# microsoft/AI2BMD

Hardware: NVIDIA H100
Metric: MD steps/sec (higher is better)
Workload: dtype f32

## Files before the change

### ai2bmd_b200/csrc/k_edge_tc.cuh

```cuda
#pragma once
#include "k_edge.cuh"
#include "tc_common.cuh"

namespace vb {

constexpr int TC_TE = 128;
constexpr int TC_STAGES = 2;
constexpr int TC_MAX_STAGES = 3;
constexpr int TC_SLABS = D / tc::SLAB_K;
static_assert((TC_SLABS & (TC_SLABS - 1)) == 0, "tc_slab rotates the slab order with a mask: TC_SLABS must be a power of two");
constexpr int TC_MAXJOBS = 12;
constexpr int TC_LT = D + LDS_PAD;
typedef float TcRow[TC_LT];

struct TcJob {
    const float* img;
    int accumulate;
};

struct TcShared {
    alignas(1024) uint8_t ring[TC_STAGES][tc::STAGE_BYTES];
    alignas(16) float tile[TC_TE][TC_LT];
    alignas(16) float abuf[TC_TE][TC_LT];
    EdgeMeta<TC_TE> meta;
// ... 29 lines not shown
    const int stage = k % NS, job = (k / TC_SLABS) % sh.njobs, s = tc_slab(k % TC_SLABS);
    const char* src = reinterpret_cast<const char*>(sh.jobs[job].img) + (size_t)s * tc::STAGE_BYTES;
    tc::mbar_arrive_expect_tx(&sh.b_full[stage], tc::STAGE_BYTES);
    tc::tma_load_1d(tc_stage_ptr(sh, stage), src, tc::STAGE_BYTES, &sh.b_full[stage]);
}

}


namespace vb {

constexpr int TC2_CWARPS = 16;
constexpr int TC2_CTHREADS = TC2_CWARPS * 32;
constexpr int TC2_THREADS = TC2_CTHREADS;
constexpr int TC2_NGRP = TC2_CTHREADS / D;

struct EdgeTcArgs {
    int layer;
    ModelW mw;
    Workspace ws;
    TcJob jobs[TC_MAXJOBS];
    int njobs;
    int tile_rows;
    unsigned long long* tl;
};
constexpr int TC_TL_SLOTS = 64;
#define TC_TL(k) do { if (a.tl != nullptr && blockIdx.x == 0 && it == 0 && threadIdx.x == 0) a.tl[k] = (unsigned long long)clock64(); } while (0)

__device__ __forceinline__ void csync() { asm volatile("bar.sync 1, %0;" ::"n"(TC2_CTHREADS) : "memory"); }

constexpr int TC2_WS_THREADS = TC2_CTHREADS / 2;
__device__ __forceinline__ bool tc2_is_mma_warp(int warp) { return ((warp >> 2) & 1) == 0; }
__device__ __forceinline__ void gather_sync() { asm volatile("bar.sync 2, %0;" ::"n"(TC2_WS_THREADS) : "memory"); }
__device__ __forceinline__ void handoff_arrive(int id) { asm volatile("bar.arrive %0, %1;" ::"r"(id), "n"(TC2_CTHREADS) : "memory"); }
__device__ __forceinline__ void handoff_wait(int id) { asm volatile("bar.sync %0, %1;" ::"r"(id), "n"(TC2_CTHREADS) : "memory"); }

template <int ROWS>
struct TcRing {
    static constexpr int NS = tc_nstages(ROWS);
    int next = 0;
};

template <int ROWS>
__device__ __forceinline__ void tc2_setup(TcShared& sh, const TcRing<ROWS>&, const TcJob* jobs, int njobs, int ntiles) {
    constexpr int NS = TcRing<ROWS>::NS;
    if (threadIdx.x == 0) {
        for (int s = 0; s < NS; s++) { tc::mbar_init(&sh.b_full[s], 1); sh.released[s] = 0; }
        tc::mbar_init(&sh.b_tile, TC2_CWARPS);
        sh.jobs = jobs; sh.njobs = njobs; sh.nslabs = ntiles * njobs * TC_SLABS;
        tc::fence_barrier_init();
    }
    __syncthreads();
    if (threadIdx.x == 0)
        for (int k = 0; k < NS; k++) tc_issue<NS>(sh, k);
}

template <int NS, int NW>
__device__ __forceinline__ void tc2_release(TcShared& sh, int k, int lane) {
    __syncwarp();
    if (lane == 0) {
        const uint32_t before = tc::atom_add_acq_rel(&sh.released[k % NS], 1u);
        if (before % NW == NW - 1) tc_issue<NS>(sh, k + NS);
    }
}

__device__ __forceinline__ void tc2_tile_to_a(TcShared& sh, int rows) {
// ... 201 lines not shown
    const int trows = min(ROWS, max(16, a.tile_rows));
    const int ntiles_total = (E + trows - 1) / trows;
    const int my_tiles = ((int)blockIdx.x < ntiles_total) ? (ntiles_total - (int)blockIdx.x + (int)gridDim.x - 1) / (int)gridDim.x : 0;
    if (a.tl != nullptr && blockIdx.x == 0 && threadIdx.x == 0) a.tl[0] = (unsigned long long)clock64();
    TcRing<ROWS> ring;
    tc2_setup(sh, ring, a.jobs, a.njobs, my_tiles);
    if (a.tl != nullptr && blockIdx.x == 0 && threadIdx.x == 0) a.tl[1] = (unsigned long long)clock64();

    float acc[32];
    const float* __restrict__ Fin = ws.F[l];
    float* __restrict__ Fout = upd ? ws.F[l + 1] : nullptr;
    const float* __restrict__ QKV = ws.QKV[l];
    const float* __restrict__ VN = ws.VN[l];
    const float* __restrict__ TU = ws.TU[l];
    float* __restrict__ P1 = ws.P1[l];
    float* __restrict__ SP = ws.SP[l];
    float* __restrict__ ATT = ws.ATT[l];
    for (int it = 0; it < my_tiles; it++) {
        const uint32_t tpar = (uint32_t)(it & 1);
        const int e0 = ((int)blockIdx.x + it * (int)gridDim.x) * trows;
        const int nvalid = min(trows, E - e0);
        {
            constexpr int RW = ROWS / TC2_CWARPS;
            const int w0 = warp * RW, wn = max(0, min(RW, nvalid - w0));
            if (lane == 0) {
                if (wn > 0) tc::mbar_arrive_expect_tx(&sh.b_tile, (uint32_t)wn * D * 4);
                else tc::mbar_arrive(&sh.b_tile);
            }
            __syncwarp();
            if (lane < wn) tc::tma_load_1d(&sh.abuf[w0 + lane][0], Fin + (size_t)(e0 + w0 + lane) * D, D * 4, &sh.b_tile);
        }
        load_edge_meta<TC_TE, TC2_CTHREADS>(sh.meta, ws, e0, nvalid);
        if constexpr (SMALL) {
            enum : int { H_DK = 3, H_ATT, H_DV, H_F, H_M, H_EU };
            TcRow* const xb = tc_aux(sh);
            csync();
            if (tc2_is_mma_warp(warp)) {
                tc::mbar_wait(&sh.b_tile, tpar);
                TC_TL(2);
                tc2_mma<ROWS, true>(sh, ring, sh.abuf, acc, a.jobs[J_DK].accumulate, warp, lane, nvalid);
                tc2_acc_to(sh.tile, acc, warp, lane, nvalid);
                handoff_arrive(H_DK);
                TC_TL(4);
                tc2_mma<ROWS, true>(sh, ring, sh.abuf, acc, a.jobs[J_DV].accumulate, warp, lane, nvalid);
                TC_TL(7);
                handoff_wait(H_ATT);
                tc2_acc_to(xb, acc, warp, lane, nvalid);
                handoff_arrive(H_DV);
                TC_TL(8);
                if (upd) {
                    tc2_mma<ROWS, true>(sh, ring, sh.abuf, acc, a.jobs[J_F].accumulate, warp, lane, nvalid);
                    tc2_acc_to(sh.tile, acc, warp, lane, nvalid);
                    handoff_arrive(H_F);
                    TC_TL(11);
                }
                handoff_wait(H_M);
                TC_TL(3);
                tc2_mma<ROWS, true>(sh, ring, xb, acc, a.jobs[J_S1].accumulate, warp, lane, nvalid);
                tc2_acc_to(sh.abuf, acc, warp, lane, nvalid);
                TC_TL(13);
                if (threadIdx.x == 0 && it + 1 < my_tiles) {
                    const int en = ((int)blockIdx.x + (it + 1) * (int)gridDim.x) * trows;
                    tc::tma_prefetch_l2(Fin + (size_t)en * D, (uint32_t)min(trows, E - en) * D * 4);
                }
                tc2_mma<ROWS, true>(sh, ring, xb, acc, a.jobs[J_S2].accumulate, warp, lane, nvalid);
                TC_TL(16);
                if (upd) handoff_wait(H_EU);
// ... 197 lines not shown
            }
            TC_TL(12);
            float bnd[2][3] = {{0.f, 0.f, 0.f}, {0.f, 0.f, 0.f}};
            tc2_mma(sh, ring, sh.abuf, acc, a.jobs[J_S1].accumulate, warp, lane, nvalid);
            TC_TL(13);
            csync();
            tc2_acc_to(sh.tile, acc, warp, lane, nvalid);
            csync();
            TC_TL(14);
            tc_fwd_s1(sh, ws, lw, VN, SP, sh.tile, e0, nvalid, cch, grp, TC2_NGRP, bnd);
            TC_TL(15);
            if (threadIdx.x == 0 && it + 1 < my_tiles) {
                const int en = ((int)blockIdx.x + (it + 1) * (int)gridDim.x) * trows;
                tc::tma_prefetch_l2(Fin + (size_t)en * D, (uint32_t)min(trows, E - en) * D * 4);
            }
            tc2_mma(sh, ring, sh.abuf, acc, a.jobs[J_S2].accumulate, warp, lane, nvalid);
            TC_TL(16);
            csync();
            tc2_acc_to(sh.tile, acc, warp, lane, nvalid);
            csync();
            TC_TL(17);
            tc_fwd_s2(sh, ws, lw, SP, sh.tile, e0, nvalid, cch, grp, TC2_NGRP, bnd);
            TC_TL(18);
        }
        csync();
    }
    if (a.tl != nullptr && blockIdx.x == 0 && threadIdx.x == 0) a.tl[31] = (unsigned long long)clock64();
}

}

namespace vb {

template <int ROWS>
__global__ void __launch_bounds__(TC2_THREADS, 1) edge_bwd_tc_kernel(const __grid_constant__ EdgeTcArgs a) {
    pdl_entry();
    extern __shared__ __align__(1024) uint8_t dyn_raw[];
    TcShared& sh = *tc_shared_base(dyn_raw);
    const Workspace& ws = a.ws;
    const int l = a.layer;
    const bool upd = (l < L - 1);
    const int J_G3A = 0, J_G3B = 1, J_G4DV = 2, J_G4DK = 3, J_G4F = 4;
    const int J_LAST = upd ? J_G4F : J_G4DK;
    constexpr int RPW = ROWS / TC2_CWARPS;
    constexpr int RB4 = (RPW % 4 == 0) ? 4 : 2;
    constexpr bool SMALL = ROWS <= 64;
    constexpr int RBM = SMALL ? 2 : RB4;
    const int warp = threadIdx.x >> 5, lane = threadIdx.x & 31, col = lane * 4, hd = lane >> 2;
    const int E = ws.rowptr[ws.N];
    const int trows = min(ROWS, max(16, a.tile_rows));
    const int ntiles_total = (E + trows - 1) / trows;
    const int my_tiles = ((int)blockIdx.x < ntiles_total) ? (ntiles_total - (int)blockIdx.x + (int)gridDim.x - 1) / (int)gridDim.x : 0;
    if (a.tl != nullptr && blockIdx.x == 0 && threadIdx.x == 0) a.tl[0] = (unsigned long long)clock64();
    TcRing<ROWS> ring;
    tc2_setup(sh, ring, a.jobs, a.njobs, my_tiles);
    if (a.tl != nullptr && blockIdx.x == 0 && threadIdx.x == 0) a.tl[1] = (unsigned long long)clock64();

    float acc[32];
    const float* __restrict__ QKV = ws.QKV[l];
    const float* __restrict__ VN = ws.VN[l];
    const float* __restrict__ TU = ws.TU[l];
    const float* __restrict__ P1 = ws.P1[l];
    const float* __restrict__ SP = ws.SP[l];
    const float* __restrict__ ATT = ws.ATT[l];
    const int cch = threadIdx.x & (D - 1), grp = threadIdx.x >> 7;
    for (int it = 0; it < my_tiles; it++) {
        const int e0 = ((int)blockIdx.x + it * (int)gridDim.x) * trows;
        const int nvalid = min(trows, E - e0);
        const int rpw = (nvalid + TC2_CWARPS - 1) / TC2_CWARPS, r0 = warp * rpw;
        load_edge_meta<TC_TE, TC2_CTHREADS>(sh.meta, ws, e0, nvalid);
        csync();
        TC_TL(2);
        if constexpr (SMALL) {
#pragma unroll 1
            for (int rb = 0; rb < RPW; rb += RB4) {
                if (rb >= rpw) break;
                float4 sp[RB4][2], gM[RB4][3], vn[RB4][3];
#pragma unroll
                for (int u = 0; u < RB4; u++) {
                    const int row = r0 + rb + u;
                    const size_t e = (size_t)(e0 + ((rb + u < rpw && row < nvalid) ? row : 0));
                    const size_t i3 = (size_t)sh.meta.dst[row] * 3, j3 = (size_t)sh.meta.src[row] * 3;
                    sp[u][0] = ldg4(SP + e * 2 * D + col);
                    sp[u][1] = ldg4(SP + e * 2 * D + D + col);
#pragma unroll
                    for (int s = 0; s < 3; s++) { gM[u][s] = ldg4(ws.GVEC + (i3 + s) * D + col); vn[u][s] = ldg4(VN + (j3 + s) * D + col); }
                }
#pragma unroll
                for (int u = 0; u < RB4; u++) {
                    const int row = r0 + rb + u;
                    const bool mine = rb + u < rpw, ok = (mine && row < nvalid);
                    const size_t j3 = (size_t)sh.meta.src[row] * 3;
                    const float4 dd = sh.meta.d[row];
                    const float4 s1 = silu4(sp[u][0]), s2 = silu4(sp[u][1]);
                    const float4 gs1 = gM[u][0] * vn[u][0] + gM[u][1] * vn[u][1] + gM[u][2] * vn[u][2];
                    const float gx_ = warp_sum(hsum4(gM[u][0] * s2)), gy_ = warp_sum(hsum4(gM[u][1] * s2)), gz_ = warp_sum(hsum4(gM[u][2] * s2));
                    if (mine) {
                        st4(&sh.abuf[row][col], ok ? gs1 * dsilu4(sp[u][0]) : f4s(0.f));
                        st4(&sh.tile[row][col], ok ? (gM[u][0] * dd.x + gM[u][1] * dd.y + gM[u][2] * dd.z) * dsilu4(sp[u][1]) : f4s(0.f));
                        if (lane == 0) { sh.eacc[row][1] = gx_; sh.eacc[row][2] = gy_; sh.eacc[row][3] = gz_; }
                    }
                    if (ok) {
                        red4(ws.GVNMSG + (j3 + 0) * D + col, gM[u][0] * s1);
                        red4(ws.GVNMSG + (j3 + 1) * D + col, gM[u][1] * s1);
                        red4(ws.GVNMSG + (j3 + 2) * D + col, gM[u][2] * s1);
                    }
                }
            }
            TC_TL(3);
        } else {
#pragma unroll 1
            for (int rb = 0; rb < RPW; rb += RB4) {
                if (rb >= rpw) break;
                float4 sp[RB4], gM[RB4][3], vn[RB4][3];
#pragma unroll
                for (int u = 0; u < RB4; u++) {
                    const int row = r0 + rb + u;
                    const size_t e = (size_t)(e0 + ((rb + u < rpw && row < nvalid) ? row : 0));
                    const size_t i3 = (size_t)sh.meta.dst[row] * 3, j3 = (size_t)sh.meta.src[row] * 3;
                    sp[u] = ldg4(SP + e * 2 * D + col);
#pragma unroll
                    for (int s = 0; s < 3; s++) { gM[u][s] = ldg4(ws.GVEC + (i3 + s) * D + col); vn[u][s] = ldg4(VN + (j3 + s) * D + col); }
                }
#pragma unroll
                for (int u = 0; u < RB4; u++) {
                    const int row = r0 + rb + u;
                    const bool ok = (rb + u < rpw && row < nvalid);
                    const size_t j3 = (size_t)sh.meta.src[row] * 3;
                    const float4 s1 = silu4(sp[u]);
                    const float4 gs1 = gM[u][0] * vn[u][0] + gM[u][1] * vn[u][1] + gM[u][2] * vn[u][2];
                    if (rb + u < rpw) st4(&sh.abuf[row][col], ok ? gs1 * dsilu4(sp[u]) : f4s(0.f));
                    if (ok) {
                        red4(ws.GVNMSG + (j3 + 0) * D + col, gM[u][0] * s1);
                        red4(ws.GVNMSG + (j3 + 1) * D + col, gM[u][1] * s1);
                        red4(ws.GVNMSG + (j3 + 2) * D + col, gM[u][2] * s1);
                    }
                }
            }
            TC_TL(3);
#pragma unroll 4
            for (int r = 0; r < RPW; r++) {
                if (r >= rpw) break;
                const int row = r0 + r;
                const bool ok = (r < rpw && row < nvalid);
                const size_t e = (size_t)(e0 + (ok ? row : 0));
                const size_t i3 = (size_t)sh.meta.dst[row] * 3;
                const float4 dd = sh.meta.d[row];
                const float4 sp = ldg4(SP + e * 2 * D + D + col);
                const float4 s2 = silu4(sp);
                const float4 gM0 = ldg4(ws.GVEC + (i3 + 0) * D + col), gM1 = ldg4(ws.GVEC + (i3 + 1) * D + col),
                             gM2 = ldg4(ws.GVEC + (i3 + 2) * D + col);
                const float gx_ = warp_sum(hsum4(gM0 * s2)), gy_ = warp_sum(hsum4(gM1 * s2)), gz_ = warp_sum(hsum4(gM2 * s2));
                if (lane == 0) { sh.eacc[row][1] = gx_; sh.eacc[row][2] = gy_; sh.eacc[row][3] = gz_; }
                st4(&sh.tile[row][col], ok ? (gM0 * dd.x + gM1 * dd.y + gM2 * dd.z) * dsilu4(sp) : f4s(0.f));
            }
            TC_TL(5);
        }
        csync();
        tc2_mma(sh, ring, sh.abuf, acc, a.jobs[J_G3A].accumulate, warp, lane, nvalid);
        TC_TL(6);
        if constexpr (!SMALL) {
            tc2_tile_to_a(sh, nvalid);
            TC_TL(7);
        }
        tc2_mma(sh, ring, SMALL ? sh.tile : sh.abuf, acc, a.jobs[J_G3B].accumulate, warp, lane, nvalid);
        TC_TL(8);
        csync();
        tc2_acc_to(sh.tile, acc, warp, lane, nvalid);
        csync();
        TC_TL(9);
#pragma unroll 1
        for (int rb = 0; rb < RPW; rb += RBM) {
            if (rb >= rpw) break;
            float4 gxa[RBM], vjr[RBM], pdvr[RBM];
            float avr[RBM];
#pragma unroll
            for (int u = 0; u < RBM; u++) {
                const int row = r0 + rb + u;
                const size_t e = (size_t)(e0 + ((rb + u < rpw && row < nvalid) ? row : 0));
                gxa[u] = load_gxa(ws, (size_t)sh.meta.dst[row], col);
                vjr[u] = ldg4(QKV + (size_t)sh.meta.src[row] * 3 * D + 2 * D + col);
                pdvr[u] = ldg4(P1 + e * 3 * D + D + col);
                avr[u] = (rb + u < rpw && row < nvalid) ? __ldg(ATT + e * H + hd) : 0.f;
            }
#pragma unroll
            for (int u = 0; u < RBM; u++) {
                const int row = r0 + rb + u;
                const bool ok = (rb + u < rpw && row < nvalid);
                const size_t j = sh.meta.src[row];
                const float Ce = sh.meta.C[row];
                const float av = avr[u], sa = silu_(av), A = sa * Ce;
                const bool mine = rb + u < rpw;
                const float4 gm = mine ? ld4(&sh.tile[row][col]) + gxa[u] : f4s(0.f);
                const float4 dv = silu4(pdvr[u]);
                if (mine) st4(&sh.abuf[row][col], ok ? gm * vjr[u] * A * dsilu4(pdvr[u]) : f4s(0.f));
                const float gA = quad_sum(hsum4(gm * vjr[u] * dv));
                if (mine && (lane & 3) == 0) sh.gattn[row][hd] = gA * Ce * dsilu_(av);
                const float gc = warp_sum((lane & 3) == 0 ? gA * sa : 0.f);
                if (mine && lane == 0) sh.eacc[row][0] = gc;
                if (ok) red4(ws.GQKV + j * 3 * D + 2 * D + col, gm * dv * A);
            }
        }
        TC_TL(10);
        csync();
#pragma unroll 1
        for (int rb = 0; rb < RPW; rb += RB4) {
            if (rb >= rpw) break;
            float4 pdkr[RB4], qir[RB4], kjr[RB4];
#pragma unroll
            for (int u = 0; u < RB4; u++) {
                const int row = r0 + rb + u;
                const size_t e = (size_t)(e0 + ((rb + u < rpw && row < nvalid) ? row : 0));
                pdkr[u] = ldg4(P1 + e * 3 * D + col);
                qir[u] = ldg4(QKV + (size_t)sh.meta.dst[row] * 3 * D + col);
                kjr[u] = ldg4(QKV + (size_t)sh.meta.src[row] * 3 * D + D + col);
            }
#pragma unroll
            for (int u = 0; u < RB4; u++) {
                const int row = r0 + rb + u;
                const bool ok = (rb + u < rpw && row < nvalid);
                const size_t j = sh.meta.src[row];
                const float4 dk = silu4(pdkr[u]);
                const float gav = sh.gattn[row][hd];
                if (rb + u < rpw) st4(&sh.tile[row][col], ok ? qir[u] * kjr[u] * gav * dsilu4(pdkr[u]) : f4s(0.f));
                if (SMALL && rb + u < rpw) st4(&tc_aux(sh)[row][col], kjr[u] * dk * gav);
                if (ok) red4(ws.GQKV + j * 3 * D + D + col, qir[u] * dk * gav);
            }
        }
        TC_TL(12);
        csync();
        tc2_mma(sh, ring, sh.abuf, acc, a.jobs[J_G4DV].accumulate, warp, lane, nvalid);
        TC_TL(13);
        if constexpr (!SMALL) {
            tc2_tile_to_a(sh, nvalid);
            TC_TL(14);
            csync();
#pragma unroll 4
            for (int r = 0; r < RPW; r++) {
                if (r >= rpw) break;
                const int row = r0 + r;
                const size_t e = (size_t)(e0 + ((r < rpw && row < nvalid) ? row : 0));
                const float4 dk = silu4(ldg4(P1 + e * 3 * D + col));
                const float4 kj = ldg4(QKV + (size_t)sh.meta.src[row] * 3 * D + D + col);
                st4(&sh.tile[row][col], kj * dk * sh.gattn[row][hd]);
            }
            csync();
        }
        {
            const TcRow* const gqb = SMALL ? tc_aux(sh) : sh.tile;
            const int i_first = sh.meta.dst[0], i_last = sh.meta.dst[nvalid - 1];
            for (int i = i_first + grp; i <= i_last; i += TC2_NGRP) {
                const int q0 = ws.rowptr[i], q1 = ws.rowptr[i + 1];
                const int lo = max(q0, e0) - e0, hi = min(q1, e0 + nvalid) - e0;
                float gq = 0.f;
                for (int r = lo; r < hi; r++) gq += gqb[r][cch];
                if (q0 >= e0 && q1 <= e0 + nvalid) ws.GQKV[(size_t)i * 3 * D + cch] = gq;
                else atomicAdd(ws.GQKV + (size_t)i * 3 * D + cch, gq);
            }
        }
        TC_TL(15);
        if (upd) {
            TcRow* const gpfb = SMALL ? sh.abuf : sh.tile;
            csync();
#pragma unroll 1
            for (int rb = 0; rb < RPW; rb += 2) {
                if (rb >= rpw) break;
                float4 gfr[2], pfr[2], tir[2][3], ujr[2][3];
#pragma unroll
                for (int u = 0; u < 2; u++) {
                    const int row = r0 + rb + u;
                    const bool ok = (rb + u < rpw && row < nvalid);
                    const size_t e = (size_t)(e0 + (ok ? row : 0));
                    const size_t i3 = (size_t)sh.meta.dst[row] * 3, j3 = (size_t)sh.meta.src[row] * 3;
                    gfr[u] = ok ? ld4(ws.GF + e * D + col) : f4s(0.f);
                    pfr[u] = ldg4(P1 + e * 3 * D + 2 * D + col);
#pragma unroll
                    for (int s = 0; s < 3; s++) {
                        tir[u][s] = ldg4(TU + (i3 + s) * 2 * D + col);
                        ujr[u][s] = ldg4(TU + (j3 + s) * 2 * D + D + col);
                    }
                }
#pragma unroll
                for (int u = 0; u < 2; u++) {
                    const int row = r0 + rb + u;
                    const bool ok = (rb + u < rpw && row < nvalid);
                    const size_t e = (size_t)(e0 + (ok ? row : 0));
                    const size_t j3 = (size_t)sh.meta.src[row] * 3;
                    const float4 dd = sh.meta.d[row];
                    const float4 gfn = gfr[u], pf = pfr[u];
                    const float4 fp = silu4(pf);
                    const float dv3[3] = {dd.x, dd.y, dd.z};
                    const float4 a1 = tir[u][0] * dd.x + tir[u][1] * dd.y + tir[u][2] * dd.z;
                    const float4 a2 = ujr[u][0] * dd.x + ujr[u][1] * dd.y + ujr[u][2] * dd.z;
                    float4 w1[3], w2[3];
#pragma unroll
                    for (int s = 0; s < 3; s++) { w1[s] = tir[u][s] - a1 * dv3[s]; w2[s] = ujr[u][s] - a2 * dv3[s]; }
                    const float4 wdot = w1[0] * w2[0] + w1[1] * w2[1] + w1[2] * w2[2];
                    const float4 gwd = gfn * fp;
                    if (rb + u < rpw) {
                        st4(&gpfb[row][col], gfn * wdot * dsilu4(pf));
                        if (SMALL) st4(&tc_aux(sh)[row][col], gwd);
                    }
                    const float4 c1 = gwd * (w2[0] * dd.x + w2[1] * dd.y + w2[2] * dd.z);
                    const float4 c2 = gwd * (w1[0] * dd.x + w1[1] * dd.y + w1[2] * dd.z);
                    float gdl[3];
                    float4 gu[3];
#pragma unroll
                    for (int s = 0; s < 3; s++) {
                        const float4 gw1 = gwd * w2[s], gw2 = gwd * w1[s];
                        gu[s] = gw2 - c2 * dv3[s];
                        gdl[s] = warp_sum(hsum4(tir[u][s] * c1 + a1 * gw1 + ujr[u][s] * c2 + a2 * gw2));
                    }
                    if (lane == 0 && rb + u < rpw) { sh.eacc[row][1] -= gdl[0]; sh.eacc[row][2] -= gdl[1]; sh.eacc[row][3] -= gdl[2]; }
                    if (ok) {
                        red4(ws.GTU + (j3 + 0) * 2 * D + D + col, gu[0]);
                        red4(ws.GTU + (j3 + 1) * 2 * D + D + col, gu[1]);
                        red4(ws.GTU + (j3 + 2) * 2 * D + D + col, gu[2]);
                    }
                    (void)e;
                }
            }
            TC_TL(16);
            csync();
            tc2_mma(sh, ring, SMALL ? sh.tile : sh.abuf, acc, a.jobs[J_G4DK].accumulate, warp, lane, nvalid);
            TC_TL(17);
            if constexpr (!SMALL) {
                tc2_tile_to_a(sh, nvalid);
                TC_TL(18);
                csync();
#pragma unroll 4
                for (int r = 0; r < RPW; r++) {
                    if (r >= rpw) break;
                    const int row = r0 + r;
                    const bool ok = (r < rpw && row < nvalid);
                    const size_t e = (size_t)(e0 + (ok ? row : 0));
                    const float4 gfn = ok ? ld4(ws.GF + e * D + col) : f4s(0.f);
                    st4(&sh.tile[row][col], gfn * silu4(ldg4(P1 + e * 3 * D + 2 * D + col)));
                }
                csync();
            }
            {
                const TcRow* const gwb = SMALL ? tc_aux(sh) : sh.tile;
                const int i_first = sh.meta.dst[0], i_last = sh.meta.dst[nvalid - 1];
                for (int i = i_first + grp; i <= i_last; i += TC2_NGRP) {
                    const int q0 = ws.rowptr[i], q1 = ws.rowptr[i + 1];
                    const int lo = max(q0, e0) - e0, hi = min(q1, e0 + nvalid) - e0;
                    float gt0 = 0.f, gt1 = 0.f, gt2 = 0.f;
                    auto term = [&](int r, float u0, float u1, float u2) {
                        const float4 dd = sh.meta.d[r];
                        const float gw = gwb[r][cch];
                        const float a2 = u0 * dd.x + u1 * dd.y + u2 * dd.z;
                        const float w20 = u0 - a2 * dd.x, w21 = u1 - a2 * dd.y, w22 = u2 - a2 * dd.z;
                        const float wd = w20 * dd.x + w21 * dd.y + w22 * dd.z;
                        gt0 += gw * (w20 - wd * dd.x);
                        gt1 += gw * (w21 - wd * dd.y);
                        gt2 += gw * (w22 - wd * dd.z);
                    };
                    int r = lo;
                    for (; r + 4 <= hi; r += 4) {
                        float u[4][3];
#pragma unroll
                        for (int q = 0; q < 4; q++) {
                            const size_t j3 = (size_t)sh.meta.src[r + q] * 3;
                            u[q][0] = __ldg(TU + (j3 + 0) * 2 * D + D + cch);
                            u[q][1] = __ldg(TU + (j3 + 1) * 2 * D + D + cch);
                            u[q][2] = __ldg(TU + (j3 + 2) * 2 * D + D + cch);
                        }
#pragma unroll
                        for (int q = 0; q < 4; q++) term(r + q, u[q][0], u[q][1], u[q][2]);
                    }
                    for (; r < hi; r++) {
                        const size_t j3 = (size_t)sh.meta.src[r] * 3;
                        term(r, __ldg(TU + (j3 + 0) * 2 * D + D + cch), __ldg(TU + (j3 + 1) * 2 * D + D + cch),
                             __ldg(TU + (j3 + 2) * 2 * D + D + cch));
                    }
                    if (q0 >= e0 && q1 <= e0 + nvalid) {
                        ws.GTU[((size_t)i * 3 + 0) * 2 * D + cch] = gt0;
                        ws.GTU[((size_t)i * 3 + 1) * 2 * D + cch] = gt1;
                        ws.GTU[((size_t)i * 3 + 2) * 2 * D + cch] = gt2;
                    } else {
                        atomicAdd(ws.GTU + ((size_t)i * 3 + 0) * 2 * D + cch, gt0);
                        atomicAdd(ws.GTU + ((size_t)i * 3 + 1) * 2 * D + cch, gt1);
                        atomicAdd(ws.GTU + ((size_t)i * 3 + 2) * 2 * D + cch, gt2);
                    }
                }
            }
        }
        TC_TL(19);
        if (threadIdx.x < 3 && it + 1 < my_tiles) {
            const int en = ((int)blockIdx.x + (it + 1) * (int)gridDim.x) * trows;
            const uint32_t nn = (uint32_t)min(trows, E - en);
            if (threadIdx.x == 0) tc::tma_prefetch_l2(SP + (size_t)en * 2 * D, nn * 2 * D * 4);
            else if (threadIdx.x == 1) tc::tma_prefetch_l2(P1 + (size_t)en * 3 * D, nn * 3 * D * 4);
            else tc::tma_prefetch_l2(ATT + (size_t)en * H, nn * H * 4);
        }
        tc2_mma(sh, ring, (SMALL && !upd) ? sh.tile : sh.abuf, acc, a.jobs[J_LAST].accumulate, warp, lane, nvalid);
        TC_TL(20);
        if (!SMALL || !upd) csync();
        tc2_acc_to(sh.tile, acc, warp, lane, nvalid);
        csync();
        TC_TL(21);
#pragma unroll 4
        for (int r = 0; r < RPW; r++) {
            if (r >= rpw) break;
            const int row = r0 + r;
            if ((r < rpw && row < nvalid)) {
                float* g = ws.GF + (size_t)(e0 + row) * D + col;
                float4 v = ld4(&sh.tile[row][col]);
                if (upd) v = v + ld4(g);
                st4(g, v);
            }
        }
        if (threadIdx.x < nvalid) {
            float* ea = ws.eacc + (size_t)(e0 + threadIdx.x) * 4;
            st4(ea, ld4(ea) + ld4(&sh.eacc[threadIdx.x][0]));
        }
        TC_TL(22);
        csync();
    }
    if (a.tl != nullptr && blockIdx.x == 0 && threadIdx.x == 0) a.tl[31] = (unsigned long long)clock64();
}

}
```

Before: 1155.

## Warp-specialize small-tile edge backward: overlap MMA warps with gather/reduction warps

For small tiles, the edge backward kernel now splits warps into MMA warps and helper warps. Helper warps compute the force-gradient (gf) elementwise work while the G3 MMAs run, then run the per-node gq/gt segment reductions while the G4 MMAs run. MMA warps write GF straight from accumulator registers after a named-barrier handoff instead of going through shared memory. The per-row phases are pulled into helper functions, and a new named barrier id shifts the forward kernel's handoff ids. This adds more named barriers and ordering constraints between the two warp groups, so a sync mistake could cause races.

```diff
diff --git a/ai2bmd_b200/csrc/k_edge_tc.cuh b/ai2bmd_b200/csrc/k_edge_tc.cuh
--- a/ai2bmd_b200/csrc/k_edge_tc.cuh
+++ b/ai2bmd_b200/csrc/k_edge_tc.cuh
@@ -85,6 +85,7 @@
 constexpr int TC2_WS_THREADS = TC2_CTHREADS / 2;
 __device__ __forceinline__ bool tc2_is_mma_warp(int warp) { return ((warp >> 2) & 1) == 0; }
 __device__ __forceinline__ void gather_sync() { asm volatile("bar.sync 2, %0;" ::"n"(TC2_WS_THREADS) : "memory"); }
+__device__ __forceinline__ void mma_sync() { asm volatile("bar.sync 3, %0;" ::"n"(TC2_WS_THREADS) : "memory"); }
 __device__ __forceinline__ void handoff_arrive(int id) { asm volatile("bar.arrive %0, %1;" ::"r"(id), "n"(TC2_CTHREADS) : "memory"); }
 __device__ __forceinline__ void handoff_wait(int id) { asm volatile("bar.sync %0, %1;" ::"r"(id), "n"(TC2_CTHREADS) : "memory"); }
 
@@ -352,7 +353,7 @@
         }
         load_edge_meta<TC_TE, TC2_CTHREADS>(sh.meta, ws, e0, nvalid);
         if constexpr (SMALL) {
-            enum : int { H_DK = 3, H_ATT, H_DV, H_F, H_M, H_EU };
+            enum : int { H_DK = 4, H_ATT, H_DV, H_F, H_M, H_EU };
             TcRow* const xb = tc_aux(sh);
             csync();
             if (tc2_is_mma_warp(warp)) {
@@ -616,6 +617,200 @@
 
 namespace vb {
 
+
+template <int MAXR, int RB>
+__device__ __forceinline__ void tc_bwd_gm(TcShared& sh, const Workspace& ws, const float* __restrict__ QKV, const float* __restrict__ P1,
+                                          const float* __restrict__ ATT, int e0, int nvalid, int r0, int n, int lane) {
+    const int col = lane * 4, hd = lane >> 2;
+#pragma unroll 1
+    for (int rb = 0; rb < MAXR; rb += RB) {
+        if (rb >= n) break;
+        float4 gxa[RB], vjr[RB], pdvr[RB];
+        float avr[RB];
+#pragma unroll
+        for (int u = 0; u < RB; u++) {
+            const int row = r0 + rb + u;
+            const size_t e = (size_t)(e0 + ((rb + u < n && row < nvalid) ? row : 0));
+            gxa[u] = load_gxa(ws, (size_t)sh.meta.dst[row], col);
+            vjr[u] = ldg4(QKV + (size_t)sh.meta.src[row] * 3 * D + 2 * D + col);
+            pdvr[u] = ldg4(P1 + e * 3 * D + D + col);
+            avr[u] = (rb + u < n && row < nvalid) ? __ldg(ATT + e * H + hd) : 0.f;
+        }
+#pragma unroll
+        for (int u = 0; u < RB; u++) {
+            const int row = r0 + rb + u;
+            const bool ok = (rb + u < n && row < nvalid);
+            const size_t j = sh.meta.src[row];
+            const float Ce = sh.meta.C[row];
+            const float av = avr[u], sa = silu_(av), A = sa * Ce;
+            const bool mine = rb + u < n;
+            const float4 gm = mine ? ld4(&sh.tile[row][col]) + gxa[u] : f4s(0.f);
+            const float4 dv = silu4(pdvr[u]);
+            if (mine) st4(&sh.abuf[row][col], ok ? gm * vjr[u] * A * dsilu4(pdvr[u]) : f4s(0.f));
+            const float gA = quad_sum(hsum4(gm * vjr[u] * dv));
+            if (mine && (lane & 3) == 0) sh.gattn[row][hd] = gA * Ce * dsilu_(av);
+            const float gc = warp_sum((lane & 3) == 0 ? gA * sa : 0.f);
+            if (mine && lane == 0) sh.eacc[row][0] = gc;
+            if (ok) red4(ws.GQKV + j * 3 * D + 2 * D + col, gm * dv * A);
+        }
+    }
+}
+
+template <int MAXR, int RB>
+__device__ __forceinline__ void tc_bwd_gdk(TcShared& sh, const Workspace& ws, const float* __restrict__ QKV, const float* __restrict__ P1,
+                                           int e0, int nvalid, int r0, int n, int lane) {
+    const int col = lane * 4, hd = lane >> 2;
+#pragma unroll 1
+    for (int rb = 0; rb < MAXR; rb += RB) {
+        if (rb >= n) break;
+        float4 pdkr[RB], qir[RB], kjr[RB];
+#pragma unroll
+        for (int u = 0; u < RB; u++) {
+            const int row = r0 + rb + u;
+            const size_t e = (size_t)(e0 + ((rb + u < n && row < nvalid) ? row : 0));
+            pdkr[u] = ldg4(P1 + e * 3 * D + col);
+            qir[u] = ldg4(QKV + (size_t)sh.meta.dst[row] * 3 * D + col);
+            kjr[u] = ldg4(QKV + (size_t)sh.meta.src[row] * 3 * D + D + col);
+        }
+#pragma unroll
+        for (int u = 0; u < RB; u++) {
+            const int row = r0 + rb + u;
+            const bool ok = (rb + u < n && row < nvalid);
+            const size_t j = sh.meta.src[row];
+            const float4 dk = silu4(pdkr[u]);
+            const float gav = sh.gattn[row][hd];
+            if (rb + u < n) st4(&sh.tile[row][col], ok ? qir[u] * kjr[u] * gav * dsilu4(pdkr[u]) : f4s(0.f));
+            if (ok) red4(ws.GQKV + j * 3 * D + D + col, qir[u] * dk * gav);
+        }
+    }
+}
+
+template <int MAXR>
+__device__ __forceinline__ void tc_bwd_gf(TcShared& sh, const Workspace& ws, const float* __restrict__ TU, const float* __restrict__ P1,
+                                          TcRow* gpfb, int e0, int nvalid, int r0, int n, int lane) {
+    const int col = lane * 4;
+#pragma unroll 1
+    for (int rb = 0; rb < MAXR; rb += 2) {
+        if (rb >= n) break;
+        float4 gfr[2], pfr[2], tir[2][3], ujr[2][3];
+#pragma unroll
+        for (int u = 0; u < 2; u++) {
+            const int row = r0 + rb + u;
+            const bool ok = (rb + u < n && row < nvalid);
+            const size_t e = (size_t)(e0 + (ok ? row : 0));
+            const size_t i3 = (size_t)sh.meta.dst[row] * 3, j3 = (size_t)sh.meta.src[row] * 3;
+            gfr[u] = ok ? ld4(ws.GF + e * D + col) : f4s(0.f);
+            pfr[u] = ldg4(P1 + e * 3 * D + 2 * D + col);
+#pragma unroll
+            for (int s = 0; s < 3; s++) {
+                tir[u][s] = ldg4(TU + (i3 + s) * 2 * D + col);
+                ujr[u][s] = ldg4(TU + (j3 + s) * 2 * D + D + col);
+            }
+        }
+#pragma unroll
+        for (int u = 0; u < 2; u++) {
+            const int row = r0 + rb + u;
+            const bool ok = (rb + u < n && row < nvalid);
+            const size_t j3 = (size_t)sh.meta.src[row] * 3;
+            const float4 dd = sh.meta.d[row];
+            const float4 gfn = gfr[u], pf = pfr[u];
+            const float4 fp = silu4(pf);
+            const float dv3[3] = {dd.x, dd.y, dd.z};
+            const float4 a1 = tir[u][0] * dd.x + tir[u][1] * dd.y + tir[u][2] * dd.z;
+            const float4 a2 = ujr[u][0] * dd.x + ujr[u][1] * dd.y + ujr[u][2] * dd.z;
+            float4 w1[3], w2[3];
+#pragma unroll
+            for (int s = 0; s < 3; s++) { w1[s] = tir[u][s] - a1 * dv3[s]; w2[s] = ujr[u][s] - a2 * dv3[s]; }
+            const float4 wdot = w1[0] * w2[0] + w1[1] * w2[1] + w1[2] * w2[2];
+            const float4 gwd = gfn * fp;
+            if (rb + u < n) st4(&gpfb[row][col], gfn * wdot * dsilu4(pf));
+            const float4 c1 = gwd * (w2[0] * dd.x + w2[1] * dd.y + w2[2] * dd.z);
+            const float4 c2 = gwd * (w1[0] * dd.x + w1[1] * dd.y + w1[2] * dd.z);
+            float gdl[3];
+            float4 gu[3];
+#pragma unroll
+            for (int s = 0; s < 3; s++) {
+                const float4 gw1 = gwd * w2[s], gw2 = gwd * w1[s];
+                gu[s] = gw2 - c2 * dv3[s];
+                gdl[s] = warp_sum(hsum4(tir[u][s] * c1 + a1 * gw1 + ujr[u][s] * c2 + a2 * gw2));
+            }
+            if (lane == 0 && rb + u < n) { sh.eacc[row][1] -= gdl[0]; sh.eacc[row][2] -= gdl[1]; sh.eacc[row][3] -= gdl[2]; }
+            if (ok) {
+                red4(ws.GTU + (j3 + 0) * 2 * D + D + col, gu[0]);
+                red4(ws.GTU + (j3 + 1) * 2 * D + D + col, gu[1]);
+                red4(ws.GTU + (j3 + 2) * 2 * D + D + col, gu[2]);
+            }
+        }
+    }
+}
+
+template <class Gq>
+__device__ __forceinline__ void tc_bwd_gq(const TcShared& sh, const Workspace& ws, int e0, int nvalid, int c, int grp, int ngrp, Gq gq_row) {
+    const int i_first = sh.meta.dst[0], i_last = sh.meta.dst[nvalid - 1];
+    for (int i = i_first + grp; i <= i_last; i += ngrp) {
+        const int q0 = ws.rowptr[i], q1 = ws.rowptr[i + 1];
+        const int lo = max(q0, e0) - e0, hi = min(q1, e0 + nvalid) - e0;
+        float gq = 0.f;
+        int r = lo;
+        for (; r + 4 <= hi; r += 4) {
+            float v[4];
+#pragma unroll
+            for (int q = 0; q < 4; q++) v[q] = gq_row(r + q);
+#pragma unroll
+            for (int q = 0; q < 4; q++) gq += v[q];
+        }
+        for (; r < hi; r++) gq += gq_row(r);
+        if (q0 >= e0 && q1 <= e0 + nvalid) ws.GQKV[(size_t)i * 3 * D + c] = gq;
+        else atomicAdd(ws.GQKV + (size_t)i * 3 * D + c, gq);
+    }
+}
+template <class Gw>
+__device__ __forceinline__ void tc_bwd_gt(const TcShared& sh, const Workspace& ws, const float* __restrict__ TU, int e0, int nvalid,
+                                          int c, int grp, int ngrp, Gw gw_row) {
+    const int i_first = sh.meta.dst[0], i_last = sh.meta.dst[nvalid - 1];
+    for (int i = i_first + grp; i <= i_last; i += ngrp) {
+        const int q0 = ws.rowptr[i], q1 = ws.rowptr[i + 1];
+        const int lo = max(q0, e0) - e0, hi = min(q1, e0 + nvalid) - e0;
+        float gt0 = 0.f, gt1 = 0.f, gt2 = 0.f;
+        auto term = [&](int r, float gw, float u0, float u1, float u2) {
+            const float4 dd = sh.meta.d[r];
+            const float a2 = u0 * dd.x + u1 * dd.y + u2 * dd.z;
+            const float w20 = u0 - a2 * dd.x, w21 = u1 - a2 * dd.y, w22 = u2 - a2 * dd.z;
+            const float wd = w20 * dd.x + w21 * dd.y + w22 * dd.z;
+            gt0 += gw * (w20 - wd * dd.x);
+            gt1 += gw * (w21 - wd * dd.y);
+            gt2 += gw * (w22 - wd * dd.z);
+        };
+        int r = lo;
+        for (; r + 4 <= hi; r += 4) {
+            float u[4][3], gw[4];
+#pragma unroll
+            for (int q = 0; q < 4; q++) {
+                const size_t j3 = (size_t)sh.meta.src[r + q] * 3;
+                gw[q] = gw_row(r + q);
+                u[q][0] = __ldg(TU + (j3 + 0) * 2 * D + D + c);
+                u[q][1] = __ldg(TU + (j3 + 1) * 2 * D + D + c);
+                u[q][2] = __ldg(TU + (j3 + 2) * 2 * D + D + c);
+            }
+#pragma unroll
+            for (int q = 0; q < 4; q++) term(r + q, gw[q], u[q][0], u[q][1], u[q][2]);
+        }
+        for (; r < hi; r++) {
+            const size_t j3 = (size_t)sh.meta.src[r] * 3;
+            term(r, gw_row(r), __ldg(TU + (j3 + 0) * 2 * D + D + c), __ldg(TU + (j3 + 1) * 2 * D + D + c), __ldg(TU + (j3 + 2) * 2 * D + D + c));
+        }
+        if (q0 >= e0 && q1 <= e0 + nvalid) {
+            ws.GTU[((size_t)i * 3 + 0) * 2 * D + c] = gt0;
+            ws.GTU[((size_t)i * 3 + 1) * 2 * D + c] = gt1;
+            ws.GTU[((size_t)i * 3 + 2) * 2 * D + c] = gt2;
+        } else {
+            atomicAdd(ws.GTU + ((size_t)i * 3 + 0) * 2 * D + c, gt0);
+            atomicAdd(ws.GTU + ((size_t)i * 3 + 1) * 2 * D + c, gt1);
+            atomicAdd(ws.GTU + ((size_t)i * 3 + 2) * 2 * D + c, gt2);
+        }
+    }
+}
+
 template <int ROWS>
 __global__ void __launch_bounds__(TC2_THREADS, 1) edge_bwd_tc_kernel(const __grid_constant__ EdgeTcArgs a) {
     pdl_entry();
@@ -629,8 +824,7 @@
     constexpr int RPW = ROWS / TC2_CWARPS;
     constexpr int RB4 = (RPW % 4 == 0) ? 4 : 2;
     constexpr bool SMALL = ROWS <= 64;
-    constexpr int RBM = SMALL ? 2 : RB4;
-    const int warp = threadIdx.x >> 5, lane = threadIdx.x & 31, col = lane * 4, hd = lane >> 2;
+    const int warp = threadIdx.x >> 5, lane = threadIdx.x & 31, col = lane * 4;
     const int E = ws.rowptr[ws.N];
     const int trows = min(ROWS, max(16, a.tile_rows));
     const int ntiles_total = (E + trows - 1) / trows;
@@ -647,11 +841,19 @@
     const float* __restrict__ P1 = ws.P1[l];
     const float* __restrict__ SP = ws.SP[l];
     const float* __restrict__ ATT = ws.ATT[l];
-    const int cch = threadIdx.x & (D - 1), grp = threadIdx.x >> 7;
     for (int it = 0; it < my_tiles; it++) {
         const int e0 = ((int)blockIdx.x + it * (int)gridDim.x) * trows;
         const int nvalid = min(trows, E - e0);
         const int rpw = (nvalid + TC2_CWARPS - 1) / TC2_CWARPS, r0 = warp * rpw;
+        auto prefetch_next = [&] {
+            if (threadIdx.x < 3 && it + 1 < my_tiles) {
+                const int en = ((int)blockIdx.x + (it + 1) * (int)gridDim.x) * trows;
+                const uint32_t nn = (uint32_t)min(trows, E - en);
+                if (threadIdx.x == 0) tc::tma_prefetch_l2(SP + (size_t)en * 2 * D, nn * 2 * D * 4);
+                else if (threadIdx.x == 1) tc::tma_prefetch_l2(P1 + (size_t)en * 3 * D, nn * 3 * D * 4);
+                else tc::tma_prefetch_l2(ATT + (size_t)en * H, nn * H * 4);
+            }
+        };
         load_edge_meta<TC_TE, TC2_CTHREADS>(sh.meta, ws, e0, nvalid);
         csync();
         TC_TL(2);
@@ -692,7 +894,80 @@
                 }
             }
             TC_TL(3);
+            csync();
+            const bool mma = tc2_is_mma_warp(warp);
+            enum : int { H_SUMS = 4 };
+            constexpr int GRPW = ROWS / (TC2_CWARPS / 2);
+            const int gw = (warp >> 3) * 4 + (warp & 3), gt = gw * 32 + lane;
+            if (mma) {
+                tc2_mma<ROWS, true>(sh, ring, sh.abuf, acc, a.jobs[J_G3A].accumulate, warp, lane, nvalid);
+                TC_TL(6);
+                tc2_mma<ROWS, true>(sh, ring, sh.tile, acc, a.jobs[J_G3B].accumulate, warp, lane, nvalid);
+                TC_TL(8);
+                mma_sync();
+                tc2_acc_to(sh.tile, acc, warp, lane, nvalid);
+                TC_TL(9);
+            } else if (upd) {
+                const int grpw = (nvalid + 7) / 8;
+                tc_bwd_gf<GRPW>(sh, ws, TU, P1, tc_aux(sh), e0, nvalid, gw * grpw, grpw, lane);
+                TC_TLG(0);
+            }
+            csync();
+            tc_bwd_gm<RPW, 2>(sh, ws, QKV, P1, ATT, e0, nvalid, r0, rpw, lane);
+            TC_TL(10);
+            csync();
+            tc_bwd_gdk<RPW, RB4>(sh, ws, QKV, P1, e0, nvalid, r0, rpw, lane);
+            TC_TL(12);
+            csync();
+            if (mma) {
+                tc2_mma<ROWS, true>(sh, ring, sh.abuf, acc, a.jobs[J_G4DV].accumulate, warp, lane, nvalid);
+                TC_TL(13);
+                prefetch_next();
+                tc2_mma<ROWS, true>(sh, ring, sh.tile, acc, a.jobs[J_G4DK].accumulate, warp, lane, nvalid);
+                TC_TL(17);
+                if (upd) tc2_mma<ROWS, true>(sh, ring, tc_aux(sh), acc, a.jobs[J_G4F].accumulate, warp, lane, nvalid);
+                TC_TL(20);
+                const int q = warp >> 2, rr = (q & 1) * 64 + (warp & 3) * 16 + (lane >> 2), cc = (q >> 1) * 64 + 2 * (lane & 3);
+                float2 gold[8][2];
+#pragma unroll
+                for (int i = 0; i < 8; i++)
+#pragma unroll
+                    for (int h = 0; h < 2; h++)
+                        gold[i][h] = (upd && rr + 8 * h < nvalid)
+                                         ? *reinterpret_cast<const float2*>(ws.GF + (size_t)(e0 + rr + 8 * h) * D + cc + 8 * i) : make_float2(0.f, 0.f);
+                handoff_wait(H_SUMS);
+#pragma unroll
+                for (int i = 0; i < 8; i++)
+#pragma unroll
+                    for (int h = 0; h < 2; h++)
+                        if (rr + 8 * h < nvalid) {
+                            float2 v = make_float2(acc[4 * i + 2 * h], acc[4 * i + 2 * h + 1]);
+                            if (upd) v = make_float2(v.x + gold[i][h].x, v.y + gold[i][h].y);
+                            *reinterpret_cast<float2*>(ws.GF + (size_t)(e0 + rr + 8 * h) * D + cc + 8 * i) = v;
+                        }
+                TC_TL(21);
+            } else {
+                const int c = gt & (D - 1), g = gt >> 7;
+                tc_bwd_gq(sh, ws, e0, nvalid, c, g, 2, [&](int r) {
+                    const size_t e = (size_t)(e0 + r);
+                    return __ldg(QKV + (size_t)sh.meta.src[r] * 3 * D + D + c) * silu_(__ldg(P1 + e * 3 * D + c)) * sh.gattn[r][c >> 4];
+                });
+                TC_TLG(1);
+                if (upd) {
+                    tc_bwd_gt(sh, ws, TU, e0, nvalid, c, g, 2, [&](int r) {
+                        const size_t e = (size_t)(e0 + r);
+                        return ws.GF[e * D + c] * silu_(__ldg(P1 + e * 3 * D + 2 * D + c));
+                    });
+                    TC_TLG(2);
+                }
+                handoff_arrive(H_SUMS);
+                if (gt < nvalid) {
+                    float* ea = ws.eacc + (size_t)(e0 + gt) * 4;
+                    st4(ea, ld4(ea) + ld4(&sh.eacc[gt][0]));
+                }
+            }
         } else {
+            const int cch = threadIdx.x & (D - 1), grp = threadIdx.x >> 7;
 #pragma unroll 1
             for (int rb = 0; rb < RPW; rb += RB4) {
                 if (rb >= rpw) break;
@@ -739,83 +1014,25 @@
                 st4(&sh.tile[row][col], ok ? (gM0 * dd.x + gM1 * dd.y + gM2 * dd.z) * dsilu4(sp) : f4s(0.f));
             }
             TC_TL(5);
-        }
-        csync();
-        tc2_mma(sh, ring, sh.abuf, acc, a.jobs[J_G3A].accumulate, warp, lane, nvalid);
-        TC_TL(6);
-        if constexpr (!SMALL) {
+            csync();
+            tc2_mma(sh, ring, sh.abuf, acc, a.jobs[J_G3A].accumulate, warp, lane, nvalid);
+            TC_TL(6);
             tc2_tile_to_a(sh, nvalid);
             TC_TL(7);
-        }
-        tc2_mma(sh, ring, SMALL ? sh.tile : sh.abuf, acc, a.jobs[J_G3B].accumulate, warp, lane, nvalid);
-        TC_TL(8);
-        csync();
-        tc2_acc_to(sh.tile, acc, warp, lane, nvalid);
-        csync();
-        TC_TL(9);
-#pragma unroll 1
-        for (int rb = 0; rb < RPW; rb += RBM) {
-            if (rb >= rpw) break;
-            float4 gxa[RBM], vjr[RBM], pdvr[RBM];
-            float avr[RBM];
-#pragma unroll
-            for (int u = 0; u < RBM; u++) {
-                const int row = r0 + rb + u;
-                const size_t e = (size_t)(e0 + ((rb + u < rpw && row < nvalid) ? row : 0));
-                gxa[u] = load_gxa(ws, (size_t)sh.meta.dst[row], col);
-                vjr[u] = ldg4(QKV + (size_t)sh.meta.src[row] * 3 * D + 2 * D + col);
-                pdvr[u] = ldg4(P1 + e * 3 * D + D + col);
-                avr[u] = (rb + u < rpw && row < nvalid) ? __ldg(ATT + e * H + hd) : 0.f;
-            }
-#pragma unroll
-            for (int u = 0; u < RBM; u++) {
-                const int row = r0 + rb + u;
-                const bool ok = (rb + u < rpw && row < nvalid);
-                const size_t j = sh.meta.src[row];
-                const float Ce = sh.meta.C[row];
-                const float av = avr[u], sa = silu_(av), A = sa * Ce;
-                const bool mine = rb + u < rpw;
-                const float4 gm = mine ? ld4(&sh.tile[row][col]) + gxa[u] : f4s(0.f);
-                const float4 dv = silu4(pdvr[u]);
-                if (mine) st4(&sh.abuf[row][col], ok ? gm * vjr[u] * A * dsilu4(pdvr[u]) : f4s(0.f));
-                const float gA = quad_sum(hsum4(gm * vjr[u] * dv));
-                if (mine && (lane & 3) == 0) sh.gattn[row][hd] = gA * Ce * dsilu_(av);
-                const float gc = warp_sum((lane & 3) == 0 ? gA * sa : 0.f);
-                if (mine && lane == 0) sh.eacc[row][0] = gc;
-                if (ok) red4(ws.GQKV + j * 3 * D + 2 * D + col, gm * dv * A);
-            }
-        }
-        TC_TL(10);
-        csync();
-#pragma unroll 1
-        for (int rb = 0; rb < RPW; rb += RB4) {
-            if (rb >= rpw) break;
-            float4 pdkr[RB4], qir[RB4], kjr[RB4];
-#pragma unroll
-            for (int u = 0; u < RB4; u++) {
-                const int row = r0 + rb + u;
-                const size_t e = (size_t)(e0 + ((rb + u < rpw && row < nvalid) ? row : 0));
-                pdkr[u] = ldg4(P1 + e * 3 * D + col);
-                qir[u] = ldg4(QKV + (size_t)sh.meta.dst[row] * 3 * D + col);
-                kjr[u] = ldg4(QKV + (size_t)sh.meta.src[row] * 3 * D + D + col);
-            }
-#pragma unroll
-            for (int u = 0; u < RB4; u++) {
-                const int row = r0 + rb + u;
-                const bool ok = (rb + u < rpw && row < nvalid);
-                const size_t j = sh.meta.src[row];
-                const float4 dk = silu4(pdkr[u]);
-                const float gav = sh.gattn[row][hd];
-                if (rb + u < rpw) st4(&sh.tile[row][col], ok ? qir[u] * kjr[u] * gav * dsilu4(pdkr[u]) : f4s(0.f));
-                if (SMALL && rb + u < rpw) st4(&tc_aux(sh)[row][col], kjr[u] * dk * gav);
-                if (ok) red4(ws.GQKV + j * 3 * D + D + col, qir[u] * dk * gav);
-            }
-        }
-        TC_TL(12);
-        csync();
-        tc2_mma(sh, ring, sh.abuf, acc, a.jobs[J_G4DV].accumulate, warp, lane, nvalid);
-        TC_TL(13);
-        if constexpr (!SMALL) {
+            tc2_mma(sh, ring, sh.abuf, acc, a.jobs[J_G3B].accumulate, warp, lane, nvalid);
+            TC_TL(8);
+            csync();
+            tc2_acc_to(sh.tile, acc, warp, lane, nvalid);
+            csync();
+            TC_TL(9);
+            tc_bwd_gm<RPW, RB4>(sh, ws, QKV, P1, ATT, e0, nvalid, r0, rpw, lane);
+            TC_TL(10);
+            csync();
+            tc_bwd_gdk<RPW, RB4>(sh, ws, QKV, P1, e0, nvalid, r0, rpw, lane);
+            TC_TL(12);
+            csync();
+            tc2_mma(sh, ring, sh.abuf, acc, a.jobs[J_G4DV].accumulate, warp, lane, nvalid);
+            TC_TL(13);
             tc2_tile_to_a(sh, nvalid);
             TC_TL(14);
             csync();
@@ -826,89 +1043,18 @@
                 const size_t e = (size_t)(e0 + ((r < rpw && row < nvalid) ? row : 0));
                 const float4 dk = silu4(ldg4(P1 + e * 3 * D + col));
                 const float4 kj = ldg4(QKV + (size_t)sh.meta.src[row] * 3 * D + D + col);
-                st4(&sh.tile[row][col], kj * dk * sh.gattn[row][hd]);
-            }
-            csync();
-        }
-        {
-            const TcRow* const gqb = SMALL ? tc_aux(sh) : sh.tile;
-            const int i_first = sh.meta.dst[0], i_last = sh.meta.dst[nvalid - 1];
-            for (int i = i_first + grp; i <= i_last; i += TC2_NGRP) {
-                const int q0 = ws.rowptr[i], q1 = ws.rowptr[i + 1];
-                const int lo = max(q0, e0) - e0, hi = min(q1, e0 + nvalid) - e0;
-                float gq = 0.f;
-                for (int r = lo; r < hi; r++) gq += gqb[r][cch];
-                if (q0 >= e0 && q1 <= e0 + nvalid) ws.GQKV[(size_t)i * 3 * D + cch] = gq;
-                else atomicAdd(ws.GQKV + (size_t)i * 3 * D + cch, gq);
-            }
-        }
-        TC_TL(15);
-        if (upd) {
-            TcRow* const gpfb = SMALL ? sh.abuf : sh.tile;
-            csync();
-#pragma unroll 1
-            for (int rb = 0; rb < RPW; rb += 2) {
-                if (rb >= rpw) break;
-                float4 gfr[2], pfr[2], tir[2][3], ujr[2][3];
-#pragma unroll
-                for (int u = 0; u < 2; u++) {
-                    const int row = r0 + rb + u;
-                    const bool ok = (rb + u < rpw && row < nvalid);
-                    const size_t e = (size_t)(e0 + (ok ? row : 0));
-                    const size_t i3 = (size_t)sh.meta.dst[row] * 3, j3 = (size_t)sh.meta.src[row] * 3;
-                    gfr[u] = ok ? ld4(ws.GF + e * D + col) : f4s(0.f);
-                    pfr[u] = ldg4(P1 + e * 3 * D + 2 * D + col);
-#pragma unroll
-                    for (int s = 0; s < 3; s++) {
-                        tir[u][s] = ldg4(TU + (i3 + s) * 2 * D + col);
-                        ujr[u][s] = ldg4(TU + (j3 + s) * 2 * D + D + col);
-                    }
-                }
-#pragma unroll
-                for (int u = 0; u < 2; u++) {
-                    const int row = r0 + rb + u;
-                    const bool ok = (rb + u < rpw && row < nvalid);
-                    const size_t e = (size_t)(e0 + (ok ? row : 0));
-                    const size_t j3 = (size_t)sh.meta.src[row] * 3;
-                    const float4 dd = sh.meta.d[row];
-                    const float4 gfn = gfr[u], pf = pfr[u];
-                    const float4 fp = silu4(pf);
-                    const float dv3[3] = {dd.x, dd.y, dd.z};
-                    const float4 a1 = tir[u][0] * dd.x + tir[u][1] * dd.y + tir[u][2] * dd.z;
-                    const float4 a2 = ujr[u][0] * dd.x + ujr[u][1] * dd.y + ujr[u][2] * dd.z;
-                    float4 w1[3], w2[3];
-#pragma unroll
-                    for (int s = 0; s < 3; s++) { w1[s] = tir[u][s] - a1 * dv3[s]; w2[s] = ujr[u][s] - a2 * dv3[s]; }
-                    const float4 wdot = w1[0] * w2[0] + w1[1] * w2[1] + w1[2] * w2[2];
-                    const float4 gwd = gfn * fp;
-                    if (rb + u < rpw) {
-                        st4(&gpfb[row][col], gfn * wdot * dsilu4(pf));
-                        if (SMALL) st4(&tc_aux(sh)[row][col], gwd);
-                    }
-                    const float4 c1 = gwd * (w2[0] * dd.x + w2[1] * dd.y + w2[2] * dd.z);
-                    const float4 c2 = gwd * (w1[0] * dd.x + w1[1] * dd.y + w1[2] * dd.z);
-                    float gdl[3];
-                    float4 gu[3];
-#pragma unroll
-                    for (int s = 0; s < 3; s++) {
-                        const float4 gw1 = gwd * w2[s], gw2 = gwd * w1[s];
-                        gu[s] = gw2 - c2 * dv3[s];
-                        gdl[s] = warp_sum(hsum4(tir[u][s] * c1 + a1 * gw1 + ujr[u][s] * c2 + a2 * gw2));
-                    }
-                    if (lane == 0 && rb + u < rpw) { sh.eacc[row][1] -= gdl[0]; sh.eacc[row][2] -= gdl[1]; sh.eacc[row][3] -= gdl[2]; }
-                    if (ok) {
-                        red4(ws.GTU + (j3 + 0) * 2 * D + D + col, gu[0]);
-                        red4(ws.GTU + (j3 + 1) * 2 * D + D + col, gu[1]);
-                        red4(ws.GTU + (j3 + 2) * 2 * D + D + col, gu[2]);
-                    }
-                    (void)e;
-                }
-            }
-            TC_TL(16);
-            csync();
-            tc2_mma(sh, ring, SMALL ? sh.tile : sh.abuf, acc, a.jobs[J_G4DK].accumulate, warp, lane, nvalid);
-            TC_TL(17);
-            if constexpr (!SMALL) {
+                st4(&sh.tile[row][col], kj * dk * sh.gattn[row][lane >> 2]);
+            }
+            csync();
+            tc_bwd_gq(sh, ws, e0, nvalid, cch, grp, TC2_NGRP, [&](int r) { return sh.tile[r][cch]; });
+            TC_TL(15);
+            if (upd) {
+                csync();
+                tc_bwd_gf<RPW>(sh, ws, TU, P1, sh.tile, e0, nvalid, r0, rpw, lane);
+                TC_TL(16);
+                csync();
+                tc2_mma(sh, ring, sh.abuf, acc, a.jobs[J_G4DK].accumulate, warp, lane, nvalid);
+                TC_TL(17);
                 tc2_tile_to_a(sh, nvalid);
                 TC_TL(18);
                 csync();
@@ -922,82 +1068,31 @@
                     st4(&sh.tile[row][col], gfn * silu4(ldg4(P1 + e * 3 * D + 2 * D + col)));
                 }
                 csync();
-            }
-            {
-                const TcRow* const gwb = SMALL ? tc_aux(sh) : sh.tile;
-                const int i_first = sh.meta.dst[0], i_last = sh.meta.dst[nvalid - 1];
-                for (int i = i_first + grp; i <= i_last; i += TC2_NGRP) {
-                    const int q0 = ws.rowptr[i], q1 = ws.rowptr[i + 1];
-                    const int lo = max(q0, e0) - e0, hi = min(q1, e0 + nvalid) - e0;
-                    float gt0 = 0.f, gt1 = 0.f, gt2 = 0.f;
-                    auto term = [&](int r, float u0, float u1, float u2) {
-                        const float4 dd = sh.meta.d[r];
-                        const float gw = gwb[r][cch];
-                        const float a2 = u0 * dd.x + u1 * dd.y + u2 * dd.z;
-                        const float w20 = u0 - a2 * dd.x, w21 = u1 - a2 * dd.y, w22 = u2 - a2 * dd.z;
-                        const float wd = w20 * dd.x + w21 * dd.y + w22 * dd.z;
-                        gt0 += gw * (w20 - wd * dd.x);
-                        gt1 += gw * (w21 - wd * dd.y);
-                        gt2 += gw * (w22 - wd * dd.z);
-                    };
-                    int r = lo;
-                    for (; r + 4 <= hi; r += 4) {
-                        float u[4][3];
-#pragma unroll
-                        for (int q = 0; q < 4; q++) {
-                            const size_t j3 = (size_t)sh.meta.src[r + q] * 3;
-                            u[q][0] = __ldg(TU + (j3 + 0) * 2 * D + D + cch);
-                            u[q][1] = __ldg(TU + (j3 + 1) * 2 * D + D + cch);
-                            u[q][2] = __ldg(TU + (j3 + 2) * 2 * D + D + cch);
-                        }
-#pragma unroll
-                        for (int q = 0; q < 4; q++) term(r + q, u[q][0], u[q][1], u[q][2]);
-                    }
-                    for (; r < hi; r++) {
-                        const size_t j3 = (size_t)sh.meta.src[r] * 3;
-                        term(r, __ldg(TU + (j3 + 0) * 2 * D + D + cch), __ldg(TU + (j3 + 1) * 2 * D + D + cch),
-                             __ldg(TU + (j3 + 2) * 2 * D + D + cch));
-                    }
-                    if (q0 >= e0 && q1 <= e0 + nvalid) {
-                        ws.GTU[((size_t)i * 3 + 0) * 2 * D + cch] = gt0;
-                        ws.GTU[((size_t)i * 3 + 1) * 2 * D + cch] = gt1;
-                        ws.GTU[((size_t)i * 3 + 2) * 2 * D + cch] = gt2;
-                    } else {
-                        atomicAdd(ws.GTU + ((size_t)i * 3 + 0) * 2 * D + cch, gt0);
-                        atomicAdd(ws.GTU + ((size_t)i * 3 + 1) * 2 * D + cch, gt1);
-                        atomicAdd(ws.GTU + ((size_t)i * 3 + 2) * 2 * D + cch, gt2);
-                    }
-                }
-            }
-        }
-        TC_TL(19);
-        if (threadIdx.x < 3 && it + 1 < my_tiles) {
-            const int en = ((int)blockIdx.x + (it + 1) * (int)gridDim.x) * trows;
-            const uint32_t nn = (uint32_t)min(trows, E - en);
-            if (threadIdx.x == 0) tc::tma_prefetch_l2(SP + (size_t)en * 2 * D, nn * 2 * D * 4);
-            else if (threadIdx.x == 1) tc::tma_prefetch_l2(P1 + (size_t)en * 3 * D, nn * 3 * D * 4);
-            else tc::tma_prefetch_l2(ATT + (size_t)en * H, nn * H * 4);
-        }
-        tc2_mma(sh, ring, (SMALL && !upd) ? sh.tile : sh.abuf, acc, a.jobs[J_LAST].accumulate, warp, lane, nvalid);
-        TC_TL(20);
-        if (!SMALL || !upd) csync();
-        tc2_acc_to(sh.tile, acc, warp, lane, nvalid);
-        csync();
-        TC_TL(21);
+                tc_bwd_gt(sh, ws, TU, e0, nvalid, cch, grp, TC2_NGRP, [&](int r) { return sh.tile[r][cch]; });
+            }
+            TC_TL(19);
+            prefetch_next();
+            tc2_mma(sh, ring, sh.abuf, acc, a.jobs[J_LAST].accumulate, warp, lane, nvalid);
+            TC_TL(20);
+            csync();
+            tc2_acc_to(sh.tile, acc, warp, lane, nvalid);
+            csync();
+            TC_TL(21);
 #pragma unroll 4
-        for (int r = 0; r < RPW; r++) {
-            if (r >= rpw) break;
-            const int row = r0 + r;
-            if ((r < rpw && row < nvalid)) {
-                float* g = ws.GF + (size_t)(e0 + row) * D + col;
-                float4 v = ld4(&sh.tile[row][col]);
-                if (upd) v = v + ld4(g);
-                st4(g, v);
-            }
-        }
-        if (threadIdx.x < nvalid) {
-            float* ea = ws.eacc + (size_t)(e0 + threadIdx.x) * 4;
-            st4(ea, ld4(ea) + ld4(&sh.eacc[threadIdx.x][0]));
+            for (int r = 0; r < RPW; r++) {
+                if (r >= rpw) break;
+                const int row = r0 + r;
+                if ((r < rpw && row < nvalid)) {
+                    float* g = ws.GF + (size_t)(e0 + row) * D + col;
+                    float4 v = ld4(&sh.tile[row][col]);
+                    if (upd) v = v + ld4(g);
+                    st4(g, v);
+                }
+            }
+            if (threadIdx.x < nvalid) {
+                float* ea = ws.eacc + (size_t)(e0 + threadIdx.x) * 4;
+                st4(ea, ld4(ea) + ld4(&sh.eacc[threadIdx.x][0]));
+            }
         }
         TC_TL(22);
         csync();
```

Result: faster. 1186, median of 6 (+2.6%).
